# YinkaiYu/Hybrid-Monte-Carlo-for-d-wave-SC

Hardware: AMD Instinct MI355X
Metric: fp64 leapfrog steps/sec at L=32, 1→8 MI355X; % fp64 MFMA roofline (higher is better)
Workload: dtype f64; 1 GPU; L=32 beta=16 single-chain HMC (BASELINE configs[2], C3); L=32, N=1024, bdg_dim=2048, chains_per_gpu=1, Nt=7, therm_sweeps=100, poles=12, parallelism=single GPU

## Files before the change

hybrid-monte-carlo-for-d-wave-sc_amd/csrc/dwhmc_cr.hip:

```cpp
#include <hip/hip_runtime.h>
#include <stdint.h>

#include <cmath>
#include <cstdlib>
#include <cstring>

#include "dwhmc_device.h"
#include "dwhmc_internal.h"

namespace dwh {

#ifdef CR_STAMPS
__device__ unsigned long long g_cr_stamps[kCrStampWG][32];
__device__ int g_cr_stamp_key = -1;
#define CR_STAMP_INIT(blkp) const bool stamp_on = (blkp)[0] == g_cr_stamp_key
#define CR_STAMP_AT(i, v)                                                               \
  do {                                                                                  \
    __builtin_amdgcn_sched_barrier(0);                                                  \
    const int wg_ = blockIdx.y * gridDim.x + blockIdx.x;                                \
    if (stamp_on && threadIdx.x == 0 && wg_ < kCrStampWG) g_cr_stamps[wg_][i] = (v);     \
    __builtin_amdgcn_sched_barrier(0);                                                  \
  } while (0)
#define CR_STAMP(i) CR_STAMP_AT(i, __builtin_amdgcn_s_memtime())
#define CR_RSTAMP(i) CR_STAMP_AT(i, __builtin_amdgcn_s_memrealtime())
#else
#define CR_STAMP_INIT(blkp) \
  do {                      \
  } while (0)
#define CR_STAMP_AT(i, v) \
  do {                    \
  } while (0)
#define CR_STAMP(i) \
  do {              \
  } while (0)
#define CR_RSTAMP(i) \
  do {               \
  } while (0)
#endif

#ifdef CR_GEMM_STAMPS
__device__ unsigned long long g_gemm_stamps[65536][8];
__device__ int g_gemm_sel;
#define GEMM_STAMP(i, sel)                                                             \
  do {                                                                                 \
    __builtin_amdgcn_sched_barrier(0);                                                 \
    if ((sel) && threadIdx.x == 0 && blockIdx.x < 65536)                               \
      g_gemm_stamps[blockIdx.x][i] = (i) == 0 || (i) == 6 ? __builtin_amdgcn_s_memrealtime() \
                                                          : __builtin_amdgcn_s_memtime(); \
    __builtin_amdgcn_sched_barrier(0);                                                 \
  } while (0)
#else
#define GEMM_STAMP(i, sel) \
  do {                     \
  } while (0)
#endif

__device__ __forceinline__ double2 half_delta(const double2* __restrict__ Delta, const int* __restrict__ Dsrc,
                                              int N, int c, int i, int s) {
  const int src = Dsrc[i * kSlots + s];
  if (src < 0) return make_double2(0.0, 0.0);
  const double2 d = Delta[(int64_t)c * 2 * N + src];
  return make_double2(0.5 * d.x, 0.5 * d.y);
}

__global__ __launch_bounds__(256) void k_cr_fill(double2* __restrict__ pool, int64_t item, int Lx,
                                                 int Ly, int BP, int P, int nrows, int fill_blocks,
                                                 const int* __restrict__ list,
                                                 const int* __restrict__ hcol,
                                                 const double* __restrict__ hval,
                                                 const int* __restrict__ Dcol,
                                                 const int* __restrict__ Dsrc,
                                                 const double2* __restrict__ Delta,
                                                 const double* __restrict__ ypole,
                                                 const int64_t* __restrict__ off_ph) {
  const int bi = blockIdx.y, c = bi / P, q = bi - c * P;
  const int N = Lx * Ly, HP = BP / 2;
  if ((int)blockIdx.x >= fill_blocks) {
    const int e = ((int)blockIdx.x - fill_blocks) * blockDim.x + threadIdx.x;
    if (e >= N * kSlots) return;
    const int64_t o = off_ph[e];
    if (o >= 0) pool[(int64_t)bi * item + o] = half_delta(Delta, Dsrc, N, c, e / kSlots, e % kSlots);
    return;
  }
  const int row = blockIdx.x * 4 + (threadIdx.x >> 6);
  const int lane = threadIdx.x & 63;
  if (row >= nrows) return;
  const int lb = list[row / HP], r = row - (row / HP) * HP;
  const int t = lb / Ly, y = lb - t * Ly;
  double2* out = pool + (int64_t)bi * item + ((int64_t)(t * Ly + y) * HP + r) * BP;
  const bool zero = (t == 1 && Ly < 2) || (t == 2 && Ly < 3);
  const int yr = (t == 2) ? (y + 1) % Ly : y;
  const int yc = (t == 1) ? (y + 1) % Ly : y;
  const bool rpad = r >= Lx;
  const int i = yr * Lx + r;
  int hc[kHSlots], dc[kSlots];
  double hv[kHSlots];
  double2 dv[kSlots];
#pragma unroll
  for (int s = 0; s < kHSlots; ++s) {
    hc[s] = (!rpad && !zero) ? hcol[i * kHSlots + s] : -1;
    hv[s] = (!rpad && !zero) ? hval[((int64_t)c * N + i) * kHSlots + s] : 0.0;
  }
#pragma unroll
  for (int s = 0; s < kSlots; ++s) {
    dc[s] = (!rpad && !zero) ? Dcol[i * kSlots + s] : -1;
    dv[s] = (!rpad && !zero) ? half_delta(Delta, Dsrc, N, c, i, s) : make_double2(0.0, 0.0);
  }
  const double yq = ypole[q];
  for (int cc = lane; cc < BP; cc += 64) {
    double2 v = make_double2(0.0, 0.0);
    const int pc = cc >= HP ? 1 : 0, xc = cc - pc * HP;
    if (rpad || xc >= Lx) {
      if (t == 0 && cc == r) v.x = 1.0;
    } else if (!zero) {
      const int j = yc * Lx + xc;
      if (pc == 0) {
#pragma unroll
        for (int s = 0; s < kHSlots; ++s)
          if (hc[s] == j) v.x = hv[s];
        if (i == j) v.y = -yq;
      } else {
#pragma unroll
        for (int s = 0; s < kSlots; ++s)
          if (dc[s] == j) v = dv[s];
      }
    }
    out[cc] = v;
  }
}

template <bool NEG>
__device__ __forceinline__ void mma16_3m(d4& cr, d4& ci, const double2* A, const d4& br, const d4& bi) {
  const int l = threadIdx.x & 63, lr = l & 15, lk = l >> 4;
  d4 t1 = cr, t2 = {0.0, 0.0, 0.0, 0.0}, t3 = cr + ci;
#pragma unroll
  for (int ks = 0; ks < 4; ++ks) {
    const double2 av = A[lr * 17 + 4 * ks + lk];
    const double a_r = NEG ? -av.x : av.x, a_i = NEG ? -av.y : av.y;
    t1 = __builtin_amdgcn_mfma_f64_16x16x4f64(a_r, br[ks], t1, 0, 0, 0);
    t2 = __builtin_amdgcn_mfma_f64_16x16x4f64(a_i, bi[ks], t2, 0, 0, 0);
    t3 = __builtin_amdgcn_mfma_f64_16x16x4f64(a_r + a_i, br[ks] + bi[ks], t3, 0, 0, 0);
  }
  cr = t1 - t2;
  ci = t3 - t1 - t2;
}

template <bool NEG>
__device__ __forceinline__ void mma16_3m_T(d4& cr, d4& ci, const double2* A, const d4& xr, const d4& xi) {
  const int l = threadIdx.x & 63, lr = l & 15, lk = l >> 4;
  d4 t1 = cr, t2 = {0.0, 0.0, 0.0, 0.0}, t3 = cr + ci;
#pragma unroll
  for (int ks = 0; ks < 4; ++ks) {
    const double2 bv = A[lr * 17 + 4 * ks + lk];
    const double a_r = NEG ? -xr[ks] : xr[ks], a_i = NEG ? -xi[ks] : xi[ks];
    t1 = __builtin_amdgcn_mfma_f64_16x16x4f64(a_r, bv.x, t1, 0, 0, 0);
    t2 = __builtin_amdgcn_mfma_f64_16x16x4f64(a_i, bv.y, t2, 0, 0, 0);
    t3 = __builtin_amdgcn_mfma_f64_16x16x4f64(a_r + a_i, bv.x + bv.y, t3, 0, 0, 0);
  }
  cr = t1 - t2;
  ci = t3 - t1 - t2;
}

template <int NT>
__device__ __forceinline__ void cr_inv_wg(double2* __restrict__ pool, int64_t item, int bi, int li,
                                          const int* __restrict__ blk, const int* __restrict__ dst,
                                          const int* __restrict__ slot, double* __restrict__ ldpart,
                                          int nslots, double2 (*pan)[NT][16 * 17], double* ldw) {
  constexpr int BP = 16 * NT, HP = BP / 2, TSZ = 16 * 17;
  const double2* M = pool + (int64_t)bi * item + (int64_t)blk[li] * HP * BP;
  double2* Mo = pool + (int64_t)bi * item + (int64_t)dst[li] * HP * BP;
  const int w = threadIdx.x >> 6, l = threadIdx.x & 63, lr = l & 15, lk = l >> 4;
  d4 ar[NT], ai[NT];
  CR_STAMP_INIT(blk);
  CR_RSTAMP(0);
  CR_STAMP(1);
#pragma unroll
  for (int I = 0; I < NT; ++I)
#pragma unroll
    for (int rr = 0; rr < 4; ++rr) {
      const bool diag = (I == w);
      const int row = I * 16 + (diag ? lr : lk + 4 * rr), col = w * 16 + (diag ? lk + 4 * rr : lr);
      double2 v;
      if (row < HP) {
        v = M[(int64_t)row * BP + col];
      } else {
        const double2 u = M[(int64_t)(row - HP) * BP + (col < HP ? col + HP : col - HP)];
        v = col < HP ? make_double2(u.x, -u.y) : make_double2(-u.x, u.y);
      }
      ar[I][rr] = v.x;
      ai[I][rr] = v.y;
    }
#ifdef CR_STAMPS
  if (stamp_on) __asm__ volatile("s_waitcnt vmcnt(0)" ::: "memory");
#endif
  CR_STAMP(2);
  double pp = 1.0;
  auto invert = [&](d4& tr, d4& ti) -> double {
    double2 dv[4];
#pragma unroll
    for (int jj = 0; jj < 4; ++jj) dv[jj] = make_double2(tr[jj], ti[jj]);
    const double r = wave_inv16_dpp<true>(dv);
#pragma unroll
    for (int jj = 0; jj < 4; ++jj) {
      tr[jj] = dv[jj].x;
      ti[jj] = dv[jj].y;
    }
    return r;
  };
  if (w == 0) pp = invert(ar[0], ai[0]);
  CR_STAMP(3);
#pragma unroll
  for (int kb = 0; kb < NT; ++kb) {
    double2(*P)[TSZ] = pan[kb & 1];
    double2(*Q)[TSZ] = pan[(kb + 1) & 1];
    const bool has_next = kb + 1 < NT;
    if (kb == 0 && w == 0) {
#pragma unroll
      for (int I = 0; I < NT; ++I)
#pragma unroll
        for (int rr = 0; rr < 4; ++rr) {
          const int o = (I == 0) ? lr * 17 + lk + 4 * rr : (lk + 4 * rr) * 17 + lr;
          P[I][o] = make_double2(ar[I][rr], ai[I][rr]);
        }
    }
    __syncthreads();
    CR_STAMP(4 + 3 * kb);
    d4 br = {0.0, 0.0, 0.0, 0.0}, bim = {0.0, 0.0, 0.0, 0.0};
    d4 xr = {0.0, 0.0, 0.0, 0.0}, xi = {0.0, 0.0, 0.0, 0.0};
    if (w == kb) {
#pragma unroll
      for (int rr = 0; rr < 4; ++rr) {
        const double2 v = P[kb][(lk + 4 * rr) * 17 + lr];
        br[rr] = v.x;
        bim[rr] = v.y;
      }
    } else {
      d4 tr = ar[0], ti = ai[0];
#pragma unroll
      for (int I = 1; I < NT; ++I)
        if (I == kb) {
          tr = ar[I];
          ti = ai[I];
        }
      mma16_3m<false>(xr, xi, P[kb], tr, ti);
#pragma unroll
      for (int I = 0; I < NT; ++I)
        if (I == kb) {
          ar[I] = xr;
          ai[I] = xi;
        }
      if (has_next && w == kb + 1) {
#pragma unroll
        for (int I = 0; I < NT; ++I)
          if (I != kb + 1) {
#pragma unroll
            for (int rr = 0; rr < 4; ++rr)
              Q[I][(lk + 4 * rr) * 17 + lr] = make_double2(ar[I][rr], ai[I][rr]);
          }
      }
    }
    if (has_next) __syncthreads();
    CR_STAMP(5 + 3 * kb);
    if (w == kb) {
#pragma unroll
      for (int I = 0; I < NT; ++I) {
        if (I != kb) {
          ar[I] = d4{0.0, 0.0, 0.0, 0.0};
          ai[I] = d4{0.0, 0.0, 0.0, 0.0};
          mma16_3m<true>(ar[I], ai[I], P[I], br, bim);
        } else {
          ar[I] = br;
          ai[I] = bim;
        }
      }
    } else if (has_next && w == kb + 1) {
#pragma unroll
      for (int I = 0; I < NT; ++I)
        if (I == kb + 1) {
          mma16_3m_T<true>(ar[I], ai[I], P[I], xr, xi);
          pp = invert(ar[I], ai[I]);
#pragma unroll
          for (int rr = 0; rr < 4; ++rr) Q[I][lr * 17 + lk + 4 * rr] = make_double2(ar[I][rr], ai[I][rr]);
        }
    } else {
      if (has_next) {
        d4 yr, yi, cr, ci;
#pragma unroll
        for (int rr = 0; rr < 4; ++rr) {
          const double2 v = Q[kb][(lk + 4 * rr) * 17 + lr];
          const double2 u = Q[w][(lk + 4 * rr) * 17 + lr];
          yr[rr] = v.x;
          yi[rr] = v.y;
          cr[rr] = u.x;
          ci[rr] = u.y;
        }
        mma16_3m<true>(cr, ci, P[w], yr, yi);
#pragma unroll
        for (int rr = 0; rr < 4; ++rr) Q[w][(lk + 4 * rr) * 17 + lr] = make_double2(cr[rr], ci[rr]);
      }
#pragma unroll
      for (int I = 0; I < NT; ++I)
        if (I != kb) {
          if (I == w && kb < w) mma16_3m_T<true>(ar[I], ai[I], P[I], xr, xi);
          else mma16_3m<true>(ar[I], ai[I], P[I], xr, xi);
        }
    }
    CR_STAMP(6 + 3 * kb);
  }
#pragma unroll
  for (int I = 0; I < NT / 2; ++I)
#pragma unroll
    for (int rr = 0; rr < 4; ++rr)
      Mo[(int64_t)(I * 16 + lk + 4 * rr) * BP + w * 16 + lr] = make_double2(ar[I][rr], ai[I][rr]);
  if (l == 0) ldw[w] = 0.5 * log(pp);
  __syncthreads();
  if (threadIdx.x == 0) {
    double t = 0.0;
#pragma unroll
    for (int k = 0; k < NT; ++k) t += ldw[k];
    ldpart[(int64_t)bi * nslots + slot[li]] = t;
  }
#ifdef CR_STAMPS
  if (stamp_on) __asm__ volatile("s_waitcnt vmcnt(0)" ::: "memory");
#endif
  CR_STAMP(28);
  CR_RSTAMP(30);
  CR_STAMP_AT(31, 1ull);
}

__device__ __forceinline__ void site_guard_wg(const SiteGuard& sg, int N, int c) {
  const double2* D = sg.Delta + (int64_t)c * 2 * N;
  bool over = false;
  for (int i = threadIdx.x; i < N; i += blockDim.x) {
    double sm = 0.0;
#pragma unroll
    for (int k = 0; k < 4; ++k) {
      const double2 v = D[sg.site4[4 * i + k]];
      sm += sqrt(fma(v.x, v.x, v.y * v.y));
    }
    over = over || !(sm <= sg.cap4);
  }
  if (over) *sg.flag = 1;
}

template <int NT>
__global__ __launch_bounds__(64 * NT) void k_cr_inv(double2* __restrict__ pool, int64_t item,
                                                    const int* __restrict__ blk,
                                                    const int* __restrict__ dst, int gcol,
                                                    const int* __restrict__ slot,
                                                    double* __restrict__ ldpart, int nslots,
                                                    SiteGuard sg, int N, int P) {
  __shared__ double2 pan[2][NT][16 * 17];
  __shared__ double ldw[NT];
  const int2 xy = xcd_grid2d();
  if (xy.x == gcol) {
    if (xy.y % P == 0) site_guard_wg(sg, N, xy.y / P);
    return;
  }
  cr_inv_wg<NT>(pool, item, xy.y, xy.x, blk, dst, slot, ldpart, nslots, pan, ldw);
}

__device__ __forceinline__ void tile_to_lds(double2* T, const d4& cr, const d4& ci) {
  const int l = threadIdx.x & 63, lr = l & 15, lk = l >> 4;
#pragma unroll
  for (int rr = 0; rr < 4; ++rr) T[(lk + 4 * rr) * 17 + lr] = make_double2(cr[rr], ci[rr]);
}
template <bool CONJ = false>
__device__ __forceinline__ void tile_from_lds(const double2* T, d4& cr, d4& ci) {
  const int l = threadIdx.x & 63, lr = l & 15, lk = l >> 4;
#pragma unroll
  for (int rr = 0; rr < 4; ++rr) {
    const double2 v = T[(lk + 4 * rr) * 17 + lr];
    cr[rr] = v.x;
    ci[rr] = CONJ ? -v.y : v.y;
  }
}

__device__ __forceinline__ void inv0_site_guard(const double2* __restrict__ D, const int* __restrict__ site4,
                                                int N, double cap4, int* __restrict__ flag) {
  bool over = false;
  for (int i = threadIdx.x; i < N; i += blockDim.x) {
    double sm = 0.0;
#pragma unroll
    for (int k = 0; k < 4; ++k) {
      const double2 v = D[site4[4 * i + k]];
      sm += sqrt(fma(v.x, v.x, v.y * v.y));
    }
    over = over || !(sm <= cap4);
  }
  if (over) *flag = 1;
}

__global__ __launch_bounds__(256) void k_cr_inv0(double2* __restrict__ pool, int64_t item,
                                                 const int* __restrict__ blk, const int* __restrict__ rblk,
                                                 const int* __restrict__ dst, int gcol,
                                                 const int* __restrict__ slot, double* __restrict__ ldpart,
                                                 const double* __restrict__ ldA, int nslots,
                                                 const double2* __restrict__ Delta,
                                                 const int* __restrict__ site4, int N, int P, double cap4,
                                                 int* __restrict__ flag) {
  constexpr int BP = 64, HP = 32, TSZ = 16 * 17;
  __shared__ double2 sR[4][TSZ], sB[4][TSZ], sZ[4][TSZ], sS[4][TSZ], sX[4][TSZ], sA[4][TSZ];
  __shared__ double ldw[2];
  const int2 xy = xcd_grid2d();
  const int bi = xy.y, li = xy.x;
  CR_STAMP_INIT(blk);
  CR_RSTAMP(0);
  if (li == gcol) {
    if (bi % P == 0) inv0_site_guard(Delta + (int64_t)(bi / P) * 2 * N, site4, N, cap4, flag);
    CR_RSTAMP(30);
    CR_STAMP_AT(31, 3ull);
    return;
  }
  const double2* D = pool + (int64_t)bi * item + (int64_t)blk[li] * HP * BP;
  const double2* Rm = pool + (int64_t)bi * item + (int64_t)rblk[li] * HP * BP;
  double2* Mo = pool + (int64_t)bi * item + (int64_t)dst[li] * HP * BP;
  const int w = threadIdx.x >> 6, l = threadIdx.x & 63, lr = l & 15, lk = l >> 4;
  const int ti = w >> 1, tj = w & 1;
  CR_STAMP(1);
  d4 acr, aci;
#pragma unroll
  for (int rr = 0; rr < 4; ++rr) {
    const int row = ti * 16 + lk + 4 * rr, col = tj * 16 + lr;
    const double2 a = D[(int64_t)row * BP + col];
    const double2 b = D[(int64_t)row * BP + HP + col];
    const double2 r = Rm[(int64_t)row * BP + col];
    acr[rr] = a.x;
    aci[rr] = a.y;
    sB[w][(lk + 4 * rr) * 17 + lr] = b;
    sR[w][(lk + 4 * rr) * 17 + lr] = r;
  }
  __syncthreads();
  CR_STAMP(2);
  d4 zr = {0.0, 0.0, 0.0, 0.0}, zi = {0.0, 0.0, 0.0, 0.0};
#pragma unroll
  for (int k = 0; k < 2; ++k) {
    d4 br, bim;
    tile_from_lds(sB[2 * k + tj], br, bim);
    mma16_3m<false>(zr, zi, sR[2 * ti + k], br, bim);
  }
  tile_to_lds(sZ[w], zr, zi);
  __syncthreads();
  CR_STAMP(3);
  d4 sr = acr, si = aci;
#pragma unroll
  for (int k = 0; k < 2; ++k) {
    d4 br, bim;
    tile_from_lds<true>(sZ[2 * k + tj], br, bim);
    mma16_3m<false>(sr, si, sB[2 * ti + k], br, bim);
  }
  double pp = 1.0;
  if (w == 0) pp = wave_inv16_c(sr, si);
  tile_to_lds(sS[w], sr, si);
  __syncthreads();
  CR_STAMP(4);
  d4 qr = {0.0, 0.0, 0.0, 0.0}, qi = {0.0, 0.0, 0.0, 0.0};
  if (w == 1) {
    d4 pr = {0.0, 0.0, 0.0, 0.0}, pi = {0.0, 0.0, 0.0, 0.0};
    mma16_3m<false>(pr, pi, sS[0], sr, si);
    tile_to_lds(sA[1], pr, pi);
  } else if (w == 2) {
    d4 br, bim;
    tile_from_lds(sS[0], br, bim);
    mma16_3m<false>(qr, qi, sS[2], br, bim);
    tile_to_lds(sA[2], qr, qi);
  } else if (w == 3) {
    d4 br, bim, pr = {0.0, 0.0, 0.0, 0.0}, pi = {0.0, 0.0, 0.0, 0.0};
    tile_from_lds(sS[1], br, bim);
    mma16_3m<false>(pr, pi, sS[0], br, bim);
    mma16_3m<true>(sr, si, sS[2], pr, pi);
    pp = wave_inv16_c(sr, si);
    tile_to_lds(sX[3], sr, si);
  }
  __syncthreads();
  CR_STAMP(5);
  d4 xr = sr, xi = si;
  if (w == 1) {
    d4 br, bim;
    tile_from_lds(sX[3], br, bim);
    xr = d4{0.0, 0.0, 0.0, 0.0};
    xi = d4{0.0, 0.0, 0.0, 0.0};
    mma16_3m<true>(xr, xi, sA[1], br, bim);
    tile_to_lds(sX[1], xr, xi);
  } else if (w == 2) {
    xr = d4{0.0, 0.0, 0.0, 0.0};
    xi = d4{0.0, 0.0, 0.0, 0.0};
    mma16_3m<true>(xr, xi, sX[3], qr, qi);
    tile_to_lds(sX[2], xr, xi);
  } else if (w == 0) {
    d4 br, bim, ur = {0.0, 0.0, 0.0, 0.0}, ui = {0.0, 0.0, 0.0, 0.0};
    tile_from_lds(sA[2], br, bim);
    mma16_3m<false>(ur, ui, sX[3], br, bim);
    mma16_3m<false>(xr, xi, sA[1], ur, ui);
    tile_to_lds(sX[0], xr, xi);
  }
  __syncthreads();
  CR_STAMP(6);
  d4 yr = {0.0, 0.0, 0.0, 0.0}, yi = {0.0, 0.0, 0.0, 0.0};
#pragma unroll
  for (int k = 0; k < 2; ++k) {
    d4 br, bim;
    tile_from_lds<true>(sX[2 * k + tj], br, bim);
    mma16_3m<false>(yr, yi, sZ[2 * ti + k], br, bim);
  }
  CR_STAMP(7);
#pragma unroll
  for (int rr = 0; rr < 4; ++rr) {
    const int row = ti * 16 + lk + 4 * rr, col = tj * 16 + lr;
    Mo[(int64_t)row * BP + col] = make_double2(xr[rr], xi[rr]);
    Mo[(int64_t)row * BP + HP + col] = make_double2(yr[rr], yi[rr]);
  }
  if (l == 0 && (w == 0 || w == 3)) ldw[w == 3] = 0.5 * log(pp);
  __syncthreads();
  if (threadIdx.x == 0) {
    const int64_t o = (int64_t)bi * nslots + slot[li];
    ldpart[o] = 0.5 * ldA[o] + ldw[0] + ldw[1];
  }
#ifdef CR_STAMPS
  if (stamp_on) __asm__ volatile("s_waitcnt vmcnt(0)" ::: "memory");
#endif
  CR_STAMP(28);
  CR_RSTAMP(30);
  CR_STAMP_AT(31, 1ull);
}

__global__ __launch_bounds__(576) void k_cr_inv0_96(double2* __restrict__ pool, int64_t item,
                                                    const int* __restrict__ blk, const int* __restrict__ rblk,
                                                    const int* __restrict__ dst, int gcol,
                                                    const int* __restrict__ slot, double* __restrict__ ldpart,
                                                    const double* __restrict__ ldA, int nslots,
                                                    const double2* __restrict__ Delta,
                                                    const int* __restrict__ site4, int N, int P, double cap4,
                                                    int* __restrict__ flag) {
  constexpr int BP = 96, HP = 48, TSZ = 16 * 17;
  __shared__ double2 sZ[9][TSZ], s1[9][TSZ], s2[9][TSZ], sP[TSZ];
  __shared__ double ldw[3];
  const int2 xy = xcd_grid2d();
  const int bi = xy.y, li = xy.x;
  if (li == gcol) {
    if (bi % P == 0) inv0_site_guard(Delta + (int64_t)(bi / P) * 2 * N, site4, N, cap4, flag);
    return;
  }
  const double2* D = pool + (int64_t)bi * item + (int64_t)blk[li] * HP * BP;
  const double2* Rm = pool + (int64_t)bi * item + (int64_t)rblk[li] * HP * BP;
  double2* Mo = pool + (int64_t)bi * item + (int64_t)dst[li] * HP * BP;
  const int w = threadIdx.x >> 6, l = threadIdx.x & 63, lr = l & 15, lk = l >> 4;
  const int ti = w / 3, tj = w - 3 * (w / 3);
  d4 sr, si;
#pragma unroll
  for (int rr = 0; rr < 4; ++rr) {
    const int row = ti * 16 + lk + 4 * rr, col = tj * 16 + lr;
    const double2 a = D[(int64_t)row * BP + col];
    s2[w][(lk + 4 * rr) * 17 + lr] = D[(int64_t)row * BP + HP + col];
    s1[w][(lk + 4 * rr) * 17 + lr] = Rm[(int64_t)row * BP + col];
    sr[rr] = a.x;
    si[rr] = a.y;
  }
  __syncthreads();
  d4 br, bim, zr = {0.0, 0.0, 0.0, 0.0}, zi = {0.0, 0.0, 0.0, 0.0};
#pragma unroll
  for (int k = 0; k < 3; ++k) {
    tile_from_lds(s2[3 * k + tj], br, bim);
    mma16_3m<false>(zr, zi, s1[3 * ti + k], br, bim);
  }
  tile_to_lds(sZ[w], zr, zi);
  __syncthreads();
#pragma unroll
  for (int k = 0; k < 3; ++k) {
    tile_from_lds<true>(sZ[3 * k + tj], br, bim);
    mma16_3m<false>(sr, si, s2[3 * ti + k], br, bim);
  }
  tile_to_lds(s1[w], sr, si);
  __syncthreads();
  double pp = 1.0;
#pragma unroll
  for (int p = 0; p < 3; ++p) {
    double2(*cur)[TSZ] = (p & 1) ? s2 : s1;
    double2(*nxt)[TSZ] = (p & 1) ? s1 : s2;
    if (ti == p && tj == p) {
      pp = wave_inv16_c(sr, si);
      tile_to_lds(sP, sr, si);
    }
    __syncthreads();
    if (ti == p && tj != p) {
      d4 nr = {0.0, 0.0, 0.0, 0.0}, ni = {0.0, 0.0, 0.0, 0.0};
      mma16_3m<false>(nr, ni, sP, sr, si);
      sr = nr;
      si = ni;
      tile_to_lds(cur[w], sr, si);
    }
    __syncthreads();
    if (ti != p && tj != p) {
      tile_from_lds(cur[3 * p + tj], br, bim);
      mma16_3m<true>(sr, si, cur[3 * ti + p], br, bim);
    } else if (ti != p) {
      d4 nr = {0.0, 0.0, 0.0, 0.0}, ni = {0.0, 0.0, 0.0, 0.0};
      tile_from_lds(sP, br, bim);
      mma16_3m<true>(nr, ni, cur[w], br, bim);
      sr = nr;
      si = ni;
    }
    tile_to_lds(nxt[w], sr, si);
    __syncthreads();
  }
  d4 yr = {0.0, 0.0, 0.0, 0.0}, yi = {0.0, 0.0, 0.0, 0.0};
#pragma unroll
  for (int k = 0; k < 3; ++k) {
    tile_from_lds<true>(s2[3 * k + tj], br, bim);
    mma16_3m<false>(yr, yi, sZ[3 * ti + k], br, bim);
  }
#pragma unroll
  for (int rr = 0; rr < 4; ++rr) {
    const int row = ti * 16 + lk + 4 * rr, col = tj * 16 + lr;
    Mo[(int64_t)row * BP + col] = make_double2(sr[rr], si[rr]);
    Mo[(int64_t)row * BP + HP + col] = make_double2(yr[rr], yi[rr]);
  }
  if (l == 0 && ti == tj) ldw[ti] = 0.5 * log(pp);
  __syncthreads();
  if (threadIdx.x == 0) {
    const int64_t o = (int64_t)bi * nslots + slot[li];
    ldpart[o] = 0.5 * ldA[o] + ldw[0] + ldw[1] + ldw[2];
  }
}

template <bool STATIC>
__device__ __forceinline__ void cr_inv32_wave(double2* __restrict__ pool, int64_t item, int bi, int li,
                                              const int* __restrict__ blk, const int* __restrict__ rblk,
                                              const int* __restrict__ dst, const int* __restrict__ slot,
                                              double* __restrict__ ldpart, const double* __restrict__ ldA,
                                              int nslots) {
  constexpr int BP = 32, HP = 16, TSZ = 16 * 17;
  __shared__ double2 sR[TSZ], sB[TSZ], sZ[TSZ], sX[TSZ];
  const double2* D = pool + (int64_t)bi * item + (int64_t)blk[li] * HP * BP;
  double2* Mo = pool + (int64_t)bi * item + (int64_t)dst[li] * HP * BP;
  const int l = threadIdx.x, lr = l & 15, lk = l >> 4;
  d4 sr, si;
  double ld = 0.0, pa = 1.0;
  if constexpr (STATIC) {
    const double2* Rm = pool + (int64_t)bi * item + (int64_t)rblk[li] * HP * BP;
#pragma unroll
    for (int rr = 0; rr < 4; ++rr) {
      const int row = lk + 4 * rr;
      const double2 a = D[(int64_t)row * BP + lr];
      sB[row * 17 + lr] = D[(int64_t)row * BP + HP + lr];
      sR[row * 17 + lr] = Rm[(int64_t)row * BP + lr];
      sr[rr] = a.x;
      si[rr] = a.y;
    }
    ld = 0.5 * ldA[(int64_t)bi * nslots + slot[li]];
  } else {
    d4 rr_, ri_;
#pragma unroll
    for (int rr = 0; rr < 4; ++rr) {
      const int row = lk + 4 * rr;
      const double2 a = D[(int64_t)row * BP + lr];
      sB[row * 17 + lr] = D[(int64_t)row * BP + HP + lr];
      sr[rr] = rr_[rr] = a.x;
      si[rr] = ri_[rr] = a.y;
    }
    pa = wave_inv16_c(rr_, ri_);
    tile_to_lds(sR, rr_, ri_);
  }
  __syncthreads();
  d4 br, bim, zr = {0.0, 0.0, 0.0, 0.0}, zi = {0.0, 0.0, 0.0, 0.0};
  tile_from_lds(sB, br, bim);
  mma16_3m<false>(zr, zi, sR, br, bim);
  tile_to_lds(sZ, zr, zi);
  __syncthreads();
  tile_from_lds<true>(sZ, br, bim);
  mma16_3m<false>(sr, si, sB, br, bim);
  const double ps = wave_inv16_c(sr, si);
  tile_to_lds(sX, sr, si);
  __syncthreads();
  d4 yr = {0.0, 0.0, 0.0, 0.0}, yi = {0.0, 0.0, 0.0, 0.0};
  tile_from_lds<true>(sX, br, bim);
  mma16_3m<false>(yr, yi, sZ, br, bim);
#pragma unroll
  for (int rr = 0; rr < 4; ++rr) {
    const int row = lk + 4 * rr;
    Mo[(int64_t)row * BP + lr] = make_double2(sr[rr], si[rr]);
    Mo[(int64_t)row * BP + HP + lr] = make_double2(yr[rr], yi[rr]);
  }
  if (l == 0) ldpart[(int64_t)bi * nslots + slot[li]] = ld + 0.5 * (log(pa) + log(ps));
}

__global__ __launch_bounds__(64) void k_cr_inv0_32(double2* __restrict__ pool, int64_t item,
                                                   const int* __restrict__ blk, const int* __restrict__ rblk,
                                                   const int* __restrict__ dst, int gcol,
                                                   const int* __restrict__ slot, double* __restrict__ ldpart,
                                                   const double* __restrict__ ldA, int nslots,
                                                   const double2* __restrict__ Delta,
                                                   const int* __restrict__ site4, int N, int P, double cap4,
                                                   int* __restrict__ flag) {
  const int2 xy = xcd_grid2d();
  const int bi = xy.y, li = xy.x;
  if (li == gcol) {
    if (bi % P == 0) inv0_site_guard(Delta + (int64_t)(bi / P) * 2 * N, site4, N, cap4, flag);
    return;
  }
  cr_inv32_wave<true>(pool, item, bi, li, blk, rblk, dst, slot, ldpart, ldA, nslots);
}

__global__ __launch_bounds__(64) void k_cr_inv32(double2* __restrict__ pool, int64_t item,
                                                 const int* __restrict__ blk, const int* __restrict__ dst,
                                                 int gcol, const int* __restrict__ slot,
                                                 double* __restrict__ ldpart, int nslots, SiteGuard sg, int N,
                                                 int P) {
  const int2 xy = xcd_grid2d();
  const int bi = xy.y, li = xy.x;
  if (li == gcol) {
    if (bi % P == 0) site_guard_wg(sg, N, bi / P);
    return;
  }
  cr_inv32_wave<false>(pool, item, bi, li, blk, nullptr, dst, slot, ldpart, nullptr, nslots);
}

#ifndef CR_GEMM_WAVES
#define CR_GEMM_WAVES 2
#endif
#ifndef CR_GEMM_PF
#define CR_GEMM_PF 4
#endif
constexpr int kGemmWaves = CR_GEMM_WAVES, kGemmPf = CR_GEMM_PF;
#ifndef CR_GEMM_4M
#define CR_GEMM_4M 0
#endif

__device__ __forceinline__ double flip_sign(double x, unsigned m) {
  const unsigned long long b = __builtin_bit_cast(unsigned long long, x);
  return __builtin_bit_cast(double, b ^ ((unsigned long long)m << 32));
}

template <int BP, int MI, int KSPLIT, int KQ, int PFX = 0>
__device__ __forceinline__ void cr_term(const double2* A, const double2* Bt, int c0, int crot, unsigned smask,
                                        d4 (&t1)[MI][MI], d4 (&t2)[MI][MI], d4 (&t3)[MI][MI]) {
  constexpr int HP = BP / 2, KS = BP / 4, KH = HP / 4, KSS = KS / KSPLIT, S0 = KQ * KSS;
  constexpr int PFD = PFX > 0 ? PFX : (MI == 1 ? kGemmPf : 2);
  constexpr int PF = KSS < PFD ? KSS : PFD;
  auto load = [&](int s, double2 (&a)[MI], double2 (&b)[MI]) {
#pragma unroll
    for (int mi = 0; mi < MI; ++mi) a[mi] = A[(int64_t)16 * mi * BP + s * 4];
#pragma unroll
    for (int ni = 0; ni < MI; ++ni)
      b[ni] = s < KH ? Bt[(int64_t)s * 4 * BP + c0 + 16 * ni] : Bt[(int64_t)(s - KH) * 4 * BP + crot + 16 * ni];
  };
  double2 fa[PF][MI], fb[PF][MI];
#pragma unroll
  for (int p = 0; p < PF; ++p) load(S0 + p, fa[p], fb[p]);
#pragma unroll
  for (int j = 0; j < KSS; ++j) {
    const int cs = j % PF;
    const bool syn = S0 + j >= KH;
    double ar[MI], ai[MI], br[MI], bi[MI];
#if !CR_GEMM_4M
    double as[MI], bs[MI];
#endif
#pragma unroll
    for (int mi = 0; mi < MI; ++mi) {
      ar[mi] = fa[cs][mi].x;
      ai[mi] = fa[cs][mi].y;
      if (syn) {
        const double ux = fb[cs][mi].x, uy = fb[cs][mi].y;
        br[mi] = flip_sign(ux, smask);
        bi[mi] = flip_sign(uy, smask ^ 0x80000000u);
      } else {
        br[mi] = fb[cs][mi].x;
        bi[mi] = fb[cs][mi].y;
      }
#if !CR_GEMM_4M
      as[mi] = ar[mi] + ai[mi];
      bs[mi] = syn ? flip_sign(fb[cs][mi].x - fb[cs][mi].y, smask) : br[mi] + bi[mi];
#endif
    }
    if (j + PF < KSS) load(S0 + j + PF, fa[cs], fb[cs]);
#pragma unroll
    for (int mi = 0; mi < MI; ++mi)
#pragma unroll
      for (int ni = 0; ni < MI; ++ni) {
#if CR_GEMM_4M
        t1[mi][ni] = __builtin_amdgcn_mfma_f64_16x16x4f64(ar[mi], br[ni], t1[mi][ni], 0, 0, 0);
        t3[mi][ni] = __builtin_amdgcn_mfma_f64_16x16x4f64(ar[mi], bi[ni], t3[mi][ni], 0, 0, 0);
        t2[mi][ni] = __builtin_amdgcn_mfma_f64_16x16x4f64(ai[mi], bi[ni], t2[mi][ni], 0, 0, 0);
        t3[mi][ni] = __builtin_amdgcn_mfma_f64_16x16x4f64(ai[mi], br[ni], t3[mi][ni], 0, 0, 0);
#else
        t1[mi][ni] = __builtin_amdgcn_mfma_f64_16x16x4f64(ar[mi], br[ni], t1[mi][ni], 0, 0, 0);
        t2[mi][ni] = __builtin_amdgcn_mfma_f64_16x16x4f64(ai[mi], bi[ni], t2[mi][ni], 0, 0, 0);
        t3[mi][ni] = __builtin_amdgcn_mfma_f64_16x16x4f64(as[mi], bs[ni], t3[mi][ni], 0, 0, 0);
#endif
      }
  }
}

template <int BP, int MI, int KSPLIT, int KQ, int PFX = 0>
__device__ __forceinline__ void cr_tile_part(const double2* base, const CrTask* __restrict__ tk, int tr, int tc,
                                             d4 (&t1)[MI][MI], d4 (&t2)[MI][MI], d4 (&t3)[MI][MI]) {
  constexpr int TS = 16 * MI, HP = BP / 2;
  constexpr int64_t BB = (int64_t)HP * BP;
  const int l = threadIdx.x & 63, lr = l & 15, lk = l >> 4;
  const int c0 = tc * TS, crot = c0 < HP ? c0 + HP : c0 - HP;
  const int nt = tk->nt, bq = tk->bq;
#pragma unroll 1
  for (int h = 0; h < nt; ++h) {
    const double2* A = base + tk->a[h] * BB + (int64_t)(tr * TS + lr) * BP + lk;
    const double2* Bt = base + tk->b[h] * BB + (int64_t)lk * BP + lr;
    const bool q = (bq >> h) & 1;
    const unsigned smask = ((c0 < HP) == q) ? 0x80000000u : 0u;
    cr_term<BP, MI, KSPLIT, KQ, PFX>(A, Bt, c0, crot, smask, t1, t2, t3);
  }
}

template <int BP, int MI>
__device__ __forceinline__ int64_t cr_slot_off(int v) {
  const int mi = v / (MI * 4), ni = (v / 4) % MI, rr = v % 4;
  return (int64_t)(mi * 16 + 4 * rr) * BP + ni * 16;
}

template <int BP, int MI, int KSPLIT>
__device__ __forceinline__ void cr_tile_store(d4 (&t1)[MI][MI], d4 (&t2)[MI][MI], d4 (&t3)[MI][MI], double sg,
                                              double2* O, bool hasc, const double2 (&cpf)[MI * MI * 4 / KSPLIT],
                                              bool valid, [[maybe_unused]] bool stamp = false) {
  constexpr int NV = MI * MI * 4;
  const int w = threadIdx.x >> 6, l = threadIdx.x & 63, kq = w % KSPLIT;
  auto put = [&](int v, double2 x) {
    if (hasc) {
      const double2 c = cpf[v / KSPLIT];
      x.x += c.x;
      x.y += c.y;
    }
    O[cr_slot_off<BP, MI>(v)] = x;
  };
  auto partial = [&](int v) {
    const int mi = v / (MI * 4), ni = (v / 4) % MI, rr = v % 4;
    const double a = t1[mi][ni][rr], b = t2[mi][ni][rr], c = t3[mi][ni][rr];
#if CR_GEMM_4M
    return make_double2(sg * (a - b), sg * c);
#else
    return make_double2(sg * (a - b), sg * (c - a - b));
#endif
  };
  if constexpr (KSPLIT == 1) {
    if (!valid) return;
#pragma unroll
    for (int v = 0; v < NV; ++v) put(v, partial(v));
  } else {
    __shared__ double2 red[4][NV][64];
#pragma unroll
    for (int v = 0; v < NV; ++v) red[w][v][l] = partial(v);
#ifdef CR_GEMM_STAMPS
    if (stamp) __asm__ volatile("s_waitcnt lgkmcnt(0)" ::: "memory");
    GEMM_STAMP(3, stamp);
#endif
    __syncthreads();
#ifdef CR_GEMM_STAMPS
    GEMM_STAMP(4, stamp);
#endif
    if (!valid) return;
    const int g0 = w - kq;
#pragma unroll
    for (int v = 0; v < NV; ++v) {
      if (v % KSPLIT != kq) continue;
      double2 x = red[g0][v][l];
#pragma unroll
      for (int k = 1; k < KSPLIT; ++k) {
        const double2 y = red[g0 + k][v][l];
        x.x += y.x;
        x.y += y.y;
      }
      put(v, x);
    }
  }
}

template <int BP, int MI, int KSPLIT>
__device__ __forceinline__ void cr_tile_cin(const double2* C, double2 (&cpf)[MI * MI * 4 / KSPLIT]) {
  const int kq = (threadIdx.x >> 6) % KSPLIT;
#pragma unroll
  for (int i = 0; i < MI * MI * 4 / KSPLIT; ++i) cpf[i] = C[cr_slot_off<BP, MI>(i * KSPLIT + kq)];
}

template <int BP, int MI, int KSPLIT, int PFX = 0, bool TILESIGN = false>
__device__ __forceinline__ void cr_gemm_wg(double2* __restrict__ pool, int64_t item,
                                           const CrTask* __restrict__ tasks, int ntasks, int maxt, int total,
                                           double sg, int g) {
  static_assert(MI == 2, "16 x 16 stages run k_cr_gemm16 (dispatch-ordered slots)");
  constexpr int TS = 16 * MI, TPW = 4 / KSPLIT, HP = BP / 2, NV = MI * MI * 4;
  constexpr int64_t BB = (int64_t)HP * BP;
  const int w = threadIdx.x >> 6, l = threadIdx.x & 63, lr = l & 15, lk = l >> 4;
  const int kq = w % KSPLIT;
  const int gt = __builtin_amdgcn_readfirstlane(g * TPW + w / KSPLIT);
  const int per_item = ntasks * maxt;
  const int bi = gt / per_item;
  const int rmd = gt - bi * per_item;
  bool valid = gt < total;
  const int tsk = rmd / maxt, tile = rmd - tsk * maxt;
  const CrTask* tk = tasks + (valid ? tsk : 0);
  if constexpr (TILESIGN) sg = (tk->bq & kCrNegBit) ? -1.0 : 1.0;
  const int tr0 = tk->r0 / TS, tc0 = tk->c0 / TS;
  const int ct = (tk->c1 + TS - 1) / TS - tc0;
  const int rt = (tk->r1 + TS - 1) / TS - tr0;
  valid = valid && tile < rt * ct;
  const int tr = tr0 + (valid ? tile / ct : 0);
  const int tc = tc0 + (valid ? tile % ct : 0);
  const int cin = tk->cin, out = tk->out;
  double2* base = pool + (int64_t)(valid ? bi : 0) * item;
  d4 t1[MI][MI], t2[MI][MI], t3[MI][MI];
#pragma unroll
  for (int mi = 0; mi < MI; ++mi)
#pragma unroll
    for (int ni = 0; ni < MI; ++ni) {
      t1[mi][ni] = d4{0.0, 0.0, 0.0, 0.0};
      t2[mi][ni] = d4{0.0, 0.0, 0.0, 0.0};
      t3[mi][ni] = d4{0.0, 0.0, 0.0, 0.0};
    }
  double2* O = base + out * BB + (int64_t)(tr * TS + lk) * BP + tc * TS + lr;
  const bool hasc = cin >= 0;
  double2 cpf[NV / KSPLIT];
#pragma unroll
  for (int i = 0; i < NV / KSPLIT; ++i) cpf[i] = make_double2(0.0, 0.0);
  if (hasc && valid) cr_tile_cin<BP, MI, KSPLIT>(base + cin * BB + (int64_t)(tr * TS + lk) * BP + tc * TS + lr, cpf);
  auto run = [&](auto kqc) {
    constexpr int KQ = decltype(kqc)::value;
    cr_tile_part<BP, MI, KSPLIT, KQ, PFX>(base, tk, tr, tc, t1, t2, t3);
  };
  if (valid) {
    if (KSPLIT == 1 || kq == 0) run(std::integral_constant<int, 0>{});
    if constexpr (KSPLIT >= 2) {
      if (kq == 1) run(std::integral_constant<int, 1>{});
    }
  }
  cr_tile_store<BP, MI, KSPLIT>(t1, t2, t3, sg, O, hasc, cpf, valid);
}

template <int BP, int MI, int KSPLIT>
__global__ __launch_bounds__(256) __attribute__((amdgpu_waves_per_eu(2))) void k_cr_gemm(double2* __restrict__ pool, int64_t item,
                                                 int total, double sg, int nwg, int ntasks, int maxt,
                                                 const CrTask* __restrict__ tasks) {
  cr_gemm_wg<BP, MI, KSPLIT>(pool, item, tasks, ntasks, maxt, total, sg, xcd_remap(blockIdx.x, nwg));
}

template <int BP, int KSPLIT>
__global__ __launch_bounds__(256) __attribute__((amdgpu_waves_per_eu(kGemmWaves))) void k_cr_gemm16(
    double2* __restrict__ pool, const CrSlot* __restrict__ slots, double sg) {
  constexpr int TPW = 4 / KSPLIT, NV = 4;
  const int w = __builtin_amdgcn_readfirstlane(threadIdx.x >> 6), l = threadIdx.x & 63, lr = l & 15, lk = l >> 4;
  const int kq = w % KSPLIT;
#ifdef CR_GEMM_STAMPS
  const bool g_gemm_on = (int)(gridDim.x * TPW) == g_gemm_sel;
  GEMM_STAMP(0, g_gemm_on);
  GEMM_STAMP(1, g_gemm_on);
  if (g_gemm_on && threadIdx.x == 0 && blockIdx.x < 65536)
    g_gemm_stamps[blockIdx.x][7] = __builtin_amdgcn_s_getreg((4 << 0) | (0 << 6) | (31 << 11));
#endif
  typedef uint32_t u32x16 __attribute__((ext_vector_type(16)));
  const u32x16 d = *reinterpret_cast<const u32x16*>(slots + (blockIdx.x * TPW + w / KSPLIT));
  const uint32_t out = d[2], cin = d[3];
  const bool valid = out != kCrNone;
  double2* base = pool + (((uint64_t)d[1] << 32) | d[0]);
  d4 t1[1][1], t2[1][1], t3[1][1];
  t1[0][0] = d4{0.0, 0.0, 0.0, 0.0};
  t2[0][0] = d4{0.0, 0.0, 0.0, 0.0};
  t3[0][0] = d4{0.0, 0.0, 0.0, 0.0};
#ifdef CR_GEMM_STAMPS
  if (g_gemm_on) __asm__ volatile("s_waitcnt lgkmcnt(0)" ::: "memory");
  GEMM_STAMP(2, g_gemm_on);
#endif
  const int lo = lk * BP + lr;
  const bool hasc = cin != kCrNone;
  double2 cpf[NV / KSPLIT];
#pragma unroll
  for (int i = 0; i < NV / KSPLIT; ++i) cpf[i] = make_double2(0.0, 0.0);
  if (hasc && valid) cr_tile_cin<BP, 1, KSPLIT>(base + cin + lo, cpf);
  auto run = [&](auto kqc) {
    constexpr int KQ = decltype(kqc)::value;
    const int nt = (int)d[4], rot = (int)d[14];
    uint32_t a0 = d[6], a1 = d[7], a2 = d[8], a3 = d[9], b0 = d[10], b1 = d[11], b2 = d[12], b3 = d[13];
    unsigned sm = d[5];
#pragma unroll 1
    for (int h = 0; h < nt; ++h) {
      cr_term<BP, 1, KSPLIT, KQ>(base + a0 + (lr * BP + lk), base + b0 + lo, 0, rot, (sm & 1u) << 31, t1, t2, t3);
      a0 = a1;
      a1 = a2;
      a2 = a3;
      b0 = b1;
      b1 = b2;
      b2 = b3;
      sm >>= 1;
    }
  };
  if (valid) {
    if (KSPLIT == 1 || kq == 0) run(std::integral_constant<int, 0>{});
    if constexpr (KSPLIT >= 2) {
      if (kq == 1) run(std::integral_constant<int, 1>{});
    }
    if constexpr (KSPLIT == 4) {
      if (kq == 2) run(std::integral_constant<int, 2>{});
      if (kq == 3) run(std::integral_constant<int, 3>{});
    }
  }
#ifdef CR_GEMM_STAMPS
  cr_tile_store<BP, 1, KSPLIT>(t1, t2, t3, sg, base + out + lo, hasc, cpf, valid, g_gemm_on);
#else
  cr_tile_store<BP, 1, KSPLIT>(t1, t2, t3, sg, base + out + lo, hasc, cpf, valid);
#endif
#ifdef CR_GEMM_STAMPS
  if (g_gemm_on) __asm__ volatile("s_waitcnt vmcnt(0)" ::: "memory");
  GEMM_STAMP(5, g_gemm_on);
  GEMM_STAMP(6, g_gemm_on);
#endif
}

template <int NT>
__global__ __launch_bounds__(64 * NT) void k_cr_inv_side(double2* __restrict__ pool, int64_t item,
                                                         const int* __restrict__ blk,
                                                         const int* __restrict__ dst, int ninv, int nbatch,
                                                         const int* __restrict__ slot,
                                                         double* __restrict__ ldpart, int nslots,
                                                         int nside, const CrTask* __restrict__ stasks, int nst,
                                                         int maxt, int total, SiteGuard sg, int N) {
  static_assert(NT == 4, "side work runs 4-wave workgroups");
  __shared__ double2 pan[2][NT][16 * 17];
  __shared__ double ldw[NT];
  const int b = blockIdx.x, nall = ninv * nbatch;
  if (b < nall) {
    const int bl = CR_XCD_ITEMS ? xcd_remap(b, nall) : b;
    cr_inv_wg<NT>(pool, item, bl / ninv, bl - (bl / ninv) * ninv, blk, dst, slot, ldpart, nslots, pan, ldw);
    return;
  }
  CR_STAMP_INIT(blk);
  CR_RSTAMP(0);
  if (b >= nall + nside) {
    site_guard_wg(sg, N, b - nall - nside);
    CR_RSTAMP(30);
    CR_STAMP_AT(31, 3ull);
    return;
  }
  cr_gemm_wg<16 * NT, 2, 1, 0, true>(pool, item, stasks, nst, maxt, total, 1.0, xcd_remap(b - nall, nside));
#ifdef CR_STAMPS
  if (stamp_on) __asm__ volatile("s_waitcnt vmcnt(0)" ::: "memory");
#endif
  CR_RSTAMP(30);
  CR_STAMP_AT(31, 2ull);
}

constexpr int kPfLanes = 32;
__global__ __launch_bounds__(256) void k_cr_pair_force(
    double2* __restrict__ pool, int64_t item, const int64_t* __restrict__ bond4, int N, int P,
    const double* __restrict__ cpole, double2* __restrict__ Delta, double2* __restrict__ Pair,
    double2* __restrict__ F, double2* __restrict__ Pi, double kick, double drift, double cap2,
    int* __restrict__ flag, double beta, double J) {
  constexpr int LB = kPfLanes;
  const int b = blockIdx.x * (256 / LB) + (threadIdx.x / LB), sub = threadIdx.x % LB;
  const int c = blockIdx.y;
  if (b >= 2 * N) return;
  const int64_t o1 = bond4[4 * b], o2 = bond4[4 * b + 1], p1 = bond4[4 * b + 2], p2 = bond4[4 * b + 3];
  const int64_t o = (int64_t)c * 2 * N + b;
  double2 d0 = make_double2(0.0, 0.0), p0 = make_double2(0.0, 0.0);
  if (sub == 0) {
    d0 = Delta[o];
    p0 = Pi[o];
  }
  double2 Pv = make_double2(0.0, 0.0);
  for (int q = sub; q < P; q += LB) {
    const double2* G = pool + (int64_t)(c * P + q) * item;
    const double2 g1 = G[o1], g2 = G[o2];
    const double cq = cpole[q];
    Pv.x += cq * (g1.x + g2.x);
    Pv.y += cq * (g1.y + g2.y);
  }
#pragma unroll
  for (int off = LB / 2; off > 0; off >>= 1) {
    Pv.x += __shfl_xor(Pv.x, off, LB);
    Pv.y += __shfl_xor(Pv.y, off, LB);
  }
  double2 dn = make_double2(0.0, 0.0);
  if (sub == 0) {
    Pair[o] = Pv;
    const double2 d = d0;
    const double f = -beta / (2.0 * J);
    const double2 Fv = make_double2(f * (d.x - J * Pv.x), f * (d.y - J * Pv.y));
    F[o] = Fv;
    dn = kick_drift_pre(Fv, o, p0, d0, Delta, Pi, kick, drift, cap2, flag);
  }
  if (drift != 0.0) {
    dn.x = 0.5 * __shfl(dn.x, 0, LB);
    dn.y = 0.5 * __shfl(dn.y, 0, LB);
    for (int q = sub; q < P; q += LB) {
      double2* G = pool + (int64_t)(c * P + q) * item;
      if (p1 >= 0) G[p1] = dn;
      if (p2 >= 0) G[p2] = dn;
    }
  }
}

__global__ __launch_bounds__(256) void k_cr_fermion_energy(const double2* __restrict__ pool,
                                                           int64_t item,
                                                           const int64_t* __restrict__ doff,
                                                           const double* __restrict__ ldpart,
                                                           const double* __restrict__ cpole, int N,
                                                           int nld, int P, double Cx, double beta,
                                                           double* __restrict__ part,
                                                           double* __restrict__ Ef,
                                                           double* __restrict__ Trhh,
                                                           unsigned* __restrict__ done) {
  const int q = blockIdx.x, c = blockIdx.y, bi = c * P + q;
  __shared__ double red[2][4];
  __shared__ bool last;
  const int w = threadIdx.x >> 6, l = threadIdx.x & 63;
  double ld = 0.0, t = 0.0;
  for (int k = threadIdx.x; k < nld; k += blockDim.x) ld += ldpart[(int64_t)bi * nld + k];
  for (int i = threadIdx.x; i < N; i += blockDim.x) t -= pool[(int64_t)bi * item + doff[i]].x;
  ld = wave_sum(ld);
  t = wave_sum(t);
  if (l == 0) {
    red[0][w] = ld;
    red[1][w] = t;
  }
  __syncthreads();
  if (threadIdx.x == 0) {
    part[2 * bi] = cpole[q] * (red[0][0] + red[0][1] + red[0][2] + red[0][3]);
    part[2 * bi + 1] = cpole[q] * (red[1][0] + red[1][1] + red[1][2] + red[1][3]);
    __atomic_thread_fence(__ATOMIC_RELEASE);
    const unsigned n = __hip_atomic_fetch_add(&done[c], 1u, __ATOMIC_ACQ_REL, __HIP_MEMORY_SCOPE_AGENT);
    last = (n == (unsigned)P - 1);
  }
  __syncthreads();
  if (!last || threadIdx.x != 0) return;
  __atomic_thread_fence(__ATOMIC_ACQUIRE);
  double ef = 0.0, tr = 0.0;
  for (int k = 0; k < P; ++k) {
    ef += __hip_atomic_load(&part[2 * (c * P + k)], __ATOMIC_RELAXED, __HIP_MEMORY_SCOPE_AGENT);
    tr += __hip_atomic_load(&part[2 * (c * P + k) + 1], __ATOMIC_RELAXED, __HIP_MEMORY_SCOPE_AGENT);
  }
  Ef[c] = -2.0 * N * Cx - beta * ef;
  Trhh[c] = 0.5 * N - tr;
  done[c] = 0;
}

void launch_cr_inv0(const CrDims& c, double2* pool, const int* blk, const int* rblk, const int* dst,
                    const int* slot, int n, double* ldpart, const double* ldA, hipStream_t s,
                    const double2* Delta, const int* site4, double cap4, int* flag) {
  if (n <= 0) return;
  const bool guard = Delta != nullptr && site4 != nullptr && flag != nullptr;
  hipLaunchKernelGGL(c.BP == 32 ? k_cr_inv0_32 : c.BP == 96 ? k_cr_inv0_96 : k_cr_inv0,
                     dim3(n + (guard ? 1 : 0), c.nbatch), dim3(c.BP == 32 ? 64 : c.BP == 96 ? 576 : 256), 0, s, pool,
                     c.item, blk, rblk, dst, guard ? n : -1, slot, ldpart, ldA, c.Ly, guard ? Delta : nullptr, site4,
                     c.N, c.P, cap4, flag);
}

void launch_cr_fill(const CrDims& c, double2* pool, const int* list, int nlist, const int* hcol,
                    const double* hval, const int* Dcol, const int* Dsrc, const double2* Delta,
                    const double* ypole, const int64_t* off_ph, hipStream_t s) {
  const int nrows = nlist * c.BP / 2;
  const int fill_blocks = (nrows + 3) / 4;
  const int scatter_blocks = off_ph ? (c.N * kSlots + 255) / 256 : 0;
  if (fill_blocks + scatter_blocks == 0) return;
  hipLaunchKernelGGL(k_cr_fill, dim3(fill_blocks + scatter_blocks, c.nbatch), dim3(256), 0, s, pool,
                     c.item, c.Lx, c.Ly, c.BP, c.P, nrows, fill_blocks, list, hcol, hval, Dcol, Dsrc,
                     Delta, ypole, off_ph);
}

void launch_cr_inv(const CrDims& c, double2* pool, const int* blk, const int* dst, const int* slot,
                   int n, double* ldpart, hipStream_t s, const SiteGuard& sg) {
  if (n <= 0) return;
  const bool guard = sg.Delta != nullptr;
  const dim3 g(n + (guard ? 1 : 0), c.nbatch);
  const int gcol = guard ? n : -1;
  switch (c.BP) {
    case 32:
      if (c.inv32)
        hipLaunchKernelGGL(k_cr_inv32, g, dim3(64), 0, s, pool, c.item, blk, dst, gcol, slot, ldpart, c.Ly, sg, c.N,
                           c.P);
      else
        hipLaunchKernelGGL(k_cr_inv<2>, g, dim3(128), 0, s, pool, c.item, blk, dst, gcol, slot, ldpart, c.Ly, sg,
                           c.N, c.P);
      break;
    case 64:
      hipLaunchKernelGGL(k_cr_inv<4>, g, dim3(256), 0, s, pool, c.item, blk, dst, gcol, slot, ldpart, c.Ly, sg, c.N,
                         c.P);
      break;
    case 96:
      hipLaunchKernelGGL(k_cr_inv<6>, g, dim3(384), 0, s, pool, c.item, blk, dst, gcol, slot, ldpart, c.Ly, sg, c.N,
                         c.P);
      break;
    default:
      hipLaunchKernelGGL(k_cr_inv<8>, g, dim3(512), 0, s, pool, c.item, blk, dst, gcol, slot, ldpart, c.Ly, sg, c.N,
                         c.P);
      break;
  }
}

void launch_cr_inv_side(const CrDims& c, double2* pool, const int* blk, const int* dst, const int* slot,
                        int n, double* ldpart, const CrTask* stasks, int nst, int maxt32, hipStream_t s,
                        const SiteGuard& sg) {
  if (nst <= 0) {
    launch_cr_inv(c, pool, blk, dst, slot, n, ldpart, s, sg);
    return;
  }
  const int total = c.nbatch * nst * maxt32;
  const int side_wg = (total + 3) / 4;
  const int nc = c.nbatch / c.P;
  const dim3 g(n * c.nbatch + side_wg + (sg.Delta != nullptr ? nc : 0));
  hipLaunchKernelGGL(k_cr_inv_side<4>, g, dim3(256), 0, s, pool, c.item, blk, dst, n, c.nbatch, slot, ldpart,
                     c.Ly, side_wg, stasks, nst, maxt32, total, sg, c.N);
}

void launch_cr_gemm(const CrDims& c, double2* pool, const CrTask* tasks, int ntasks, int maxt32,
                    int maxt16, const CrSlot* slots, int nslot_wgs, const CrGemmCfg& cfg, double sg,
                    hipStream_t s) {
  (void)maxt16;
  if (ntasks <= 0) return;
  const dim3 b(256);
  if (cfg.ts == 16) {
    const dim3 g(nslot_wgs);
#define CR_GEMM16(BPV, KSV) hipLaunchKernelGGL((k_cr_gemm16<BPV, KSV>), g, b, 0, s, pool, slots, sg)
#define CR_GEMM16_BP(BPV)                        \
  if (cfg.ksplit == 4) CR_GEMM16(BPV, 4);        \
  else if (cfg.ksplit == 2) CR_GEMM16(BPV, 2);   \
  else CR_GEMM16(BPV, 1);
    switch (c.BP) {
      case 32: CR_GEMM16_BP(32) break;
      case 64: CR_GEMM16_BP(64) break;
      case 96: CR_GEMM16_BP(96) break;
      default: CR_GEMM16_BP(128) break;
    }
#undef CR_GEMM16_BP
#undef CR_GEMM16
    return;
  }
  const int total = c.nbatch * ntasks * maxt32;
  const int tpw = 4 / cfg.ksplit;
  const dim3 g((total + tpw - 1) / tpw);
#define CR_GEMM(BPV, KSV) \
  hipLaunchKernelGGL((k_cr_gemm<BPV, 2, KSV>), g, b, 0, s, pool, c.item, total, sg, (int)g.x, ntasks, maxt32, tasks)
#define CR_GEMM_BP(BPV)                      \
  if (cfg.ksplit == 2) CR_GEMM(BPV, 2);      \
  else CR_GEMM(BPV, 1);
  switch (c.BP) {
    case 32: CR_GEMM_BP(32) break;
    case 64: CR_GEMM_BP(64) break;
    case 96: CR_GEMM_BP(96) break;
    default: CR_GEMM_BP(128) break;
  }
#undef CR_GEMM_BP
#undef CR_GEMM
}

void launch_cr_pair_force(const CrDims& c, double2* pool, const int64_t* bond4, const double* cpole,
                          double2* Delta, double2* Pair, double2* F, double2* Pi,
                          const KickDrift& kd, double beta, double J, hipStream_t s) {
  const int nc = c.nbatch / c.P;
  constexpr int BPW = 256 / kPfLanes;
  hipLaunchKernelGGL(k_cr_pair_force, dim3((2 * c.N + BPW - 1) / BPW, nc), dim3(256), 0, s, pool, c.item, bond4, c.N,
                     c.P, cpole, Delta, Pair, F, Pi, kd.kick, kd.drift, kd.cap * kd.cap, kd.flag, beta, J);
}

void launch_cr_fermion_energy(const CrDims& c, const double2* pool, const int64_t* doff,
                              const double* ldpart, const double* cpole, double Cx, double beta,
                              double* part, unsigned* done, double* Ef, double* Trhh, hipStream_t s) {
  const int nc = c.nbatch / c.P;
  hipLaunchKernelGGL(k_cr_fermion_energy, dim3(c.P, nc), dim3(256), 0, s, pool, c.item, doff, ldpart,
                     cpole, c.N, c.Ly, c.P, Cx, beta, part, Ef, Trhh, done);
}

}

#ifdef CR_STAMPS
namespace dwh {
int cr_stamps_arm(int key) {
  static unsigned long long zero[kCrStampWG][32];
  if (key >= 0 && hipMemcpyToSymbol(HIP_SYMBOL(g_cr_stamps), zero, sizeof(zero)) != hipSuccess) return -2;
  return hipMemcpyToSymbol(HIP_SYMBOL(g_cr_stamp_key), &key, sizeof(int)) == hipSuccess ? 0 : -2;
}
int cr_stamps_read(unsigned long long* out, int nwg) {
  if (nwg > kCrStampWG) nwg = kCrStampWG;
  return hipMemcpyFromSymbol(out, HIP_SYMBOL(g_cr_stamps), (size_t)nwg * 32 * sizeof(unsigned long long)) ==
                 hipSuccess ? 0 : -2;
}
}
#endif

#ifdef CR_GEMM_STAMPS
extern "C" int dwh_debug_gemm_stamps_select(int total) {
  return hipMemcpyToSymbol(HIP_SYMBOL(dwh::g_gemm_sel), &total, sizeof(int)) == hipSuccess ? 0 : -2;
}
extern "C" int dwh_debug_gemm_stamps_read(unsigned long long* out, int nblocks) {
  if (nblocks > 65536) nblocks = 65536;
  return hipMemcpyFromSymbol(out, HIP_SYMBOL(dwh::g_gemm_stamps), (size_t)nblocks * 8 * sizeof(unsigned long long)) ==
                 hipSuccess ? 0 : -2;
}
#endif
```

Baseline: 4155 leapfrog steps/s.

## Restructure k_cr_inv0 block inverse to rebalance waves and drop scratch tiles

```diff
diff --git a/hybrid-monte-carlo-for-d-wave-sc_amd/csrc/dwhmc_cr.hip b/hybrid-monte-carlo-for-d-wave-sc_amd/csrc/dwhmc_cr.hip
--- a/hybrid-monte-carlo-for-d-wave-sc_amd/csrc/dwhmc_cr.hip
+++ b/hybrid-monte-carlo-for-d-wave-sc_amd/csrc/dwhmc_cr.hip
@@ -400,7 +400,7 @@
                                                  const int* __restrict__ site4, int N, int P, double cap4,
                                                  int* __restrict__ flag) {
   constexpr int BP = 64, HP = 32, TSZ = 16 * 17;
-  __shared__ double2 sR[4][TSZ], sB[4][TSZ], sZ[4][TSZ], sS[4][TSZ], sX[4][TSZ], sA[4][TSZ];
+  __shared__ double2 sR[4][TSZ], sB[4][TSZ], sZ[4][TSZ], sS[4][TSZ], sX[4][TSZ], sP[TSZ];
   __shared__ double ldw[2];
   const int2 xy = xcd_grid2d();
   const int bi = xy.y, li = xy.x;
@@ -455,16 +455,30 @@
   __syncthreads();
   CR_STAMP(4);
   d4 qr = {0.0, 0.0, 0.0, 0.0}, qi = {0.0, 0.0, 0.0, 0.0};
-  if (w == 1) {
-    d4 pr = {0.0, 0.0, 0.0, 0.0}, pi = {0.0, 0.0, 0.0, 0.0};
+  d4 vr = {0.0, 0.0, 0.0, 0.0}, vi = {0.0, 0.0, 0.0, 0.0};
+  if (w == 0) {
+    const d4 ci = -si;
+    d4 ur = {0.0, 0.0, 0.0, 0.0}, ui = {0.0, 0.0, 0.0, 0.0};
+    mma16_3m<false>(vr, vi, sZ[0], sr, ci);
+    mma16_3m<false>(ur, ui, sZ[2], sr, ci);
+    tile_to_lds(sR[2], ur, ui);
+  } else if (w == 1) {
+    d4 pr = {0.0, 0.0, 0.0, 0.0}, pi = {0.0, 0.0, 0.0, 0.0}, wr, wi;
     mma16_3m<false>(pr, pi, sS[0], sr, si);
-    tile_to_lds(sA[1], pr, pi);
+    tile_to_lds(sP, pr, pi);
+    tile_from_lds(sZ[1], wr, wi);
+    mma16_3m<true>(wr, wi, sZ[0], pr, -pi);
+    tile_to_lds(sR[0], wr, wi);
   } else if (w == 2) {
-    d4 br, bim;
+    d4 br, bim, pr = {0.0, 0.0, 0.0, 0.0}, pi = {0.0, 0.0, 0.0, 0.0}, wr, wi;
     tile_from_lds(sS[0], br, bim);
     mma16_3m<false>(qr, qi, sS[2], br, bim);
-    tile_to_lds(sA[2], qr, qi);
-  } else if (w == 3) {
+    tile_from_lds(sS[1], br, bim);
+    mma16_3m<false>(pr, pi, sS[0], br, bim);
+    tile_from_lds(sZ[3], wr, wi);
+    mma16_3m<true>(wr, wi, sZ[2], pr, -pi);
+    tile_to_lds(sR[1], wr, wi);
+  } else {
     d4 br, bim, pr = {0.0, 0.0, 0.0, 0.0}, pi = {0.0, 0.0, 0.0, 0.0};
     tile_from_lds(sS[1], br, bim);
     mma16_3m<false>(pr, pi, sS[0], br, bim);
@@ -475,40 +489,47 @@
   __syncthreads();
   CR_STAMP(5);
   d4 xr = sr, xi = si;
-  if (w == 1) {
-    d4 br, bim;
-    tile_from_lds(sX[3], br, bim);
-    xr = d4{0.0, 0.0, 0.0, 0.0};
-    xi = d4{0.0, 0.0, 0.0, 0.0};
-    mma16_3m<true>(xr, xi, sA[1], br, bim);
-    tile_to_lds(sX[1], xr, xi);
-  } else if (w == 2) {
+  d4 x2r = {0.0, 0.0, 0.0, 0.0}, x2i = {0.0, 0.0, 0.0, 0.0};
+  if (w == 2) {
     xr = d4{0.0, 0.0, 0.0, 0.0};
     xi = d4{0.0, 0.0, 0.0, 0.0};
     mma16_3m<true>(xr, xi, sX[3], qr, qi);
     tile_to_lds(sX[2], xr, xi);
-  } else if (w == 0) {
-    d4 br, bim, ur = {0.0, 0.0, 0.0, 0.0}, ui = {0.0, 0.0, 0.0, 0.0};
-    tile_from_lds(sA[2], br, bim);
-    mma16_3m<false>(ur, ui, sX[3], br, bim);
-    mma16_3m<false>(xr, xi, sA[1], ur, ui);
-    tile_to_lds(sX[0], xr, xi);
+  } else if (w == 3) {
+    mma16_3m<true>(x2r, x2i, sP, sr, si);
+  } else {
+    d4 br, bim;
+    tile_from_lds<true>(sX[3], br, bim);
+    xr = d4{0.0, 0.0, 0.0, 0.0};
+    xi = d4{0.0, 0.0, 0.0, 0.0};
+    mma16_3m<false>(xr, xi, sR[1 - w], br, bim);
   }
   __syncthreads();
   CR_STAMP(6);
-  d4 yr = {0.0, 0.0, 0.0, 0.0}, yi = {0.0, 0.0, 0.0, 0.0};
-#pragma unroll
-  for (int k = 0; k < 2; ++k) {
+  if (w == 2) {
+    tile_from_lds(sS[0], x2r, x2i);
+    mma16_3m<true>(x2r, x2i, sP, xr, xi);
+  } else if (w < 2) {
     d4 br, bim;
-    tile_from_lds<true>(sX[2 * k + tj], br, bim);
-    mma16_3m<false>(yr, yi, sZ[2 * ti + k], br, bim);
+    tile_from_lds<true>(sX[2], br, bim);
+    if (w == 0) {
+      x2r = vr;
+      x2i = vi;
+    } else {
+      tile_from_lds(sR[2], x2r, x2i);
+    }
+    mma16_3m<false>(x2r, x2i, sR[w], br, bim);
   }
   CR_STAMP(7);
-#pragma unroll
-  for (int rr = 0; rr < 4; ++rr) {
-    const int row = ti * 16 + lk + 4 * rr, col = tj * 16 + lr;
-    Mo[(int64_t)row * BP + col] = make_double2(xr[rr], xi[rr]);
-    Mo[(int64_t)row * BP + HP + col] = make_double2(yr[rr], yi[rr]);
+  {
+    const int c0 = w < 2 ? HP : 0;
+    const int r1 = w == 1 ? 0 : 16, c1 = w == 2 ? 0 : 16;
+    const int r2 = w == 1 ? 16 : 0, c2 = w == 3 ? 16 : 0;
+#pragma unroll
+    for (int rr = 0; rr < 4; ++rr) {
+      Mo[(int64_t)(r1 + lk + 4 * rr) * BP + c0 + c1 + lr] = make_double2(xr[rr], xi[rr]);
+      Mo[(int64_t)(r2 + lk + 4 * rr) * BP + c0 + c2 + lr] = make_double2(x2r[rr], x2i[rr]);
+    }
   }
   if (l == 0 && (w == 0 || w == 3)) ldw[w == 3] = 0.5 * log(pp);
   __syncthreads();
```

Result: no change. 4174 leapfrog steps/s (median of 6 runs) (+0.5%).
